# yunjinli/visual-slam

Hardware: AMD Instinct MI355X
Metric: stereo frames/sec, detect+describe (1500 feats) + stereo match, 752x480 (higher is better)
Workload: dtype u8/f32/f64; 1 GPU; synthetic 752x480 stereo, 1500 feats/frame (BASELINE configs[1]); independent streams per GPU (configs[3]); inputs_resident_in_hbm=True, distinct_stereo_pairs_per_gpu=1024, distinct_scenes_per_gpu=64, stereo_frames_per_pass_per_gpu=1024, hip_streams=2, stereo_frames_per_launch=512, num_features=1500, match=threshold 70, ratio 1.2, cross-check

## Files before the change

visual-slam_amd/csrc/detect.hip:

```cpp
#include <type_traits>

#include "vsl_common.h"

#ifndef K1_ROWS
#define K1_ROWS 60
#endif
#ifndef K1_ROWS_SMALL
#define K1_ROWS_SMALL 29
#endif
#define VSL_QUALITY_LEVEL 0.01
#define K1_WLIST 384
#define K1_COLS 60

__device__ __forceinline__ int reflect101(int i, int n) { return i < 0 ? -i : (i >= n ? 2 * n - 2 - i : i); }

struct RowF {
  float rx, ry;
};

struct RowRaw {
  unsigned l, m, r;
};

typedef __amdgpu_buffer_rsrc_t ImgSrd;
__device__ __forceinline__ RowRaw rowload(ImgSrd img, int w, int yr, unsigned xm, unsigned xe, unsigned xp) {
  const int row = yr * w;
  RowRaw o;
  o.l = __builtin_amdgcn_raw_buffer_load_b8(img, (int)xm, row, 0);
  o.m = __builtin_amdgcn_raw_buffer_load_b8(img, (int)xe, row, 0);
  o.r = __builtin_amdgcn_raw_buffer_load_b8(img, (int)xp, row, 0);
  return o;
}

__device__ __forceinline__ RowF rowfilt(RowRaw p, float s, float s2) {
  const float l = (float)p.l, m = (float)p.m, r = (float)p.r;
  RowF o;
  o.rx = r - l;
  float t = s * l;
  t = t + s2 * m;
  t = t + s * r;
  o.ry = t;
  return o;
}

__device__ __forceinline__ float from_lane_below(float v) {
  return __builtin_bit_cast(float, __builtin_amdgcn_update_dpp(0, __builtin_bit_cast(int, v), 0x138, 0xf, 0xf, true));
}
__device__ __forceinline__ float from_lane_above(float v) {
  return __builtin_bit_cast(float, __builtin_amdgcn_update_dpp(0, __builtin_bit_cast(int, v), 0x130, 0xf, 0xf, true));
}

__device__ __forceinline__ double dpp_below_f64(double v) {
  const uint64_t b = __builtin_bit_cast(uint64_t, v);
  const uint32_t lo = (uint32_t)__builtin_amdgcn_update_dpp(0, (int)(uint32_t)b, 0x138, 0xf, 0xf, true);
  const uint32_t hi = (uint32_t)__builtin_amdgcn_update_dpp(0, (int)(uint32_t)(b >> 32), 0x138, 0xf, 0xf, true);
  return __builtin_bit_cast(double, ((uint64_t)hi << 32) | lo);
}

__device__ __forceinline__ double dpp_above_f64(double v) {
  const uint64_t b = __builtin_bit_cast(uint64_t, v);
  const uint32_t lo = (uint32_t)__builtin_amdgcn_update_dpp(0, (int)(uint32_t)b, 0x130, 0xf, 0xf, true);
  const uint32_t hi = (uint32_t)__builtin_amdgcn_update_dpp(0, (int)(uint32_t)(b >> 32), 0x130, 0xf, 0xf, true);
  return __builtin_bit_cast(double, ((uint64_t)hi << 32) | lo);
}

__device__ __forceinline__ float fmax3(float a, float b, float c) {
  float r;
  asm("v_max3_f32 %0, %1, %2, %3" : "=v"(r) : "v"(a), "v"(b), "v"(c));
  return r;
}

__device__ __forceinline__ float fmax2(float a, float b) {
  float r;
  asm("v_max_f32 %0, %1, %2" : "=v"(r) : "v"(a), "v"(b));
  return r;
}

#define K1_SQRT_FLOOR 0x1p-100f
__device__ __forceinline__ float fast_sqrt_rn(float t) {
  const float y = __builtin_amdgcn_rsqf(__builtin_fmaxf(t, K1_SQRT_FLOOR));
  const float r = t * y;
  const float e = __builtin_fmaf(-r, r, t);
  return __builtin_fmaf(e, 0.5f * y, r);
}
__device__ __forceinline__ float sqrt_rn(float t) {
  float r = fast_sqrt_rn(t);
  const bool small = t < K1_SQRT_FLOOR;
  if (__builtin_amdgcn_ballot_w64(small) != 0ull) {
    asm volatile("" ::: "memory");
    const bool rare = small && t > 0.f;
    if (__builtin_amdgcn_ballot_w64(rare) != 0ull) {
      asm volatile("" ::: "memory");
      if (rare) r = sqrtf(t);
    }
  }
  return r;
}

__global__ void sqrt_check_kernel(uint32_t lo, uint32_t hi, unsigned long long* bad) {
  const uint64_t stride = (uint64_t)gridDim.x * blockDim.x;
  unsigned long long n = 0;
  for (uint64_t b = (uint64_t)lo + blockIdx.x * blockDim.x + threadIdx.x; b <= hi; b += stride) {
    const float t = __builtin_bit_cast(float, (uint32_t)b);
    n += __builtin_bit_cast(uint32_t, fast_sqrt_rn(t)) != __builtin_bit_cast(uint32_t, sqrtf(t));
  }
  if (n) atomicAdd(bad, n);
}

__global__ void detect_init_kernel(int32_t* meta, int first, int n) {
  const int i = blockIdx.x * blockDim.x + threadIdx.x;
  if (i < n) {
    meta[(size_t)(first + i) * VSL_META_STRIDE + VSL_META_MAX] = INT32_MIN;
    meta[(size_t)(first + i) * VSL_META_STRIDE + VSL_META_NCAND] = 0;
  }
}

template <bool STORE_RESPONSE, int ROWS>
__global__ __launch_bounds__(256) void min_eig_response_kernel(const uint8_t* __restrict__ images,
                                                               float* __restrict__ response, int32_t* __restrict__ meta,
                                                               uint64_t* __restrict__ cand, size_t cand_cap, int w, int h,
                                                               int first, int wlist_cap, int n_images, int tiles_x, int tiles_y) {
  __shared__ uint64_t list[4][K1_WLIST];
  __shared__ int wave_n[4], wave_max[4], g_base;
  __shared__ double xbuf[4][2][66];
  const int tiles = tiles_x * tiles_y;
  int img_i, tile;
  if (n_images >= 8) {
    const int xcd = blockIdx.x & 7, sl = blockIdx.x >> 3;
    img_i = (sl / tiles) * 8 + xcd;
    tile = sl - (sl / tiles) * tiles;
  } else {
    img_i = blockIdx.x / tiles;
    tile = blockIdx.x - img_i * tiles;
  }
  if (img_i >= n_images) return;
  const int bx = tile % tiles_x, by = tile / tiles_x;
  const int slot = first + img_i;
  const ImgSrd img = __builtin_amdgcn_make_buffer_rsrc((void*)(images + (size_t)slot * w * h), 0, w * h, 0x00020000);
  float* __restrict__ resp = response + (size_t)slot * w * h;
  const int lane = threadIdx.x & 63;
  const int wave = __builtin_amdgcn_readfirstlane(threadIdx.x >> 6);
  const int xs = bx * K1_COLS;
  const int y0 = (by * 4 + wave) * ROWS;
  int n_wave = 0;
  int own_max = INT32_MIN;
  if (y0 < h) {
    const float s = (float)(1.0 / (4.0 * 3.0 * 255.0));
    const float s2 = 2.0f * s;
    const int x = xs - 2 + lane;
    const unsigned xe = (unsigned)reflect101(min(max(x, -1), w), w);
    const unsigned xm = (unsigned)reflect101((int)xe - 1, w), xp = (unsigned)reflect101((int)xe + 1, w);
    const bool own_col = lane >= 2 && lane < 2 + K1_COLS && x < w;
    const bool cand_col = own_col && x >= 1 && x < w - 1;
    const unsigned long long cand_lanes = __builtin_amdgcn_ballot_w64(cand_col);

    struct R3 {
      double xx, xy, yy;
    };
    R3 ra = {0, 0, 0}, rb = ra, bs = ra;
    float va = 0.f, vb = 0.f, hA = 0.f, hB = 0.f, hC = 0.f;
    RowF fA = {0.f, 0.f}, fB = fA, fC = fA;
    int prev_ye = -100, pre_row = -100;
    RowRaw pre = {0u, 0u, 0u};
    float vmax = -3.0e38f;
    const int y_end = min(h, y0 + ROWS);
    auto step = [&](auto steady_tag, auto even_tag, int q, R3& r2, R3& r1, float& v_mid_slot, float& v_dn_slot, float& h_up,
                    float& h_mid, float& h_dn, RowF& f0, RowF& f1, RowF& f2) {
      constexpr bool STEADY = decltype(steady_tag)::value;
      constexpr bool EVEN = decltype(even_tag)::value;
      if (STEADY) {
        f2 = rowfilt(pre, s, s2);
        pre = rowload(img, w, min(q + 2, h - 1), xm, xe, xp);
      } else {
        const int ye = reflect101(min(max(q, -1), h), h);
        if (ye == prev_ye + 1 && ye + 1 < h) {
          if (pre_row != ye + 1) pre = rowload(img, w, ye + 1, xm, xe, xp);
          f2 = rowfilt(pre, s, s2);
        } else {
          f0 = rowfilt(rowload(img, w, reflect101(ye - 1, h), xm, xe, xp), s, s2);
          f1 = rowfilt(rowload(img, w, ye, xm, xe, xp), s, s2);
          f2 = rowfilt(rowload(img, w, reflect101(ye + 1, h), xm, xe, xp), s, s2);
        }
        pre_row = min(ye + 2, h - 1);
        pre = rowload(img, w, pre_row, xm, xe, xp);
        prev_ye = ye;
      }
      const float dx = (f0.rx + f2.rx) * s + f1.rx * s2;
      const float dy = f2.ry - f0.ry;
      const double dxx = (double)(dx * dx), dxy = (double)(dx * dy), dyy = (double)(dy * dy);
      R3 cur;
      {
        xbuf[wave][0][lane + 1] = dxx;
        xbuf[wave][1][lane + 1] = dxy;
        asm volatile("" ::: "memory");
        const double lxx = xbuf[wave][0][lane], uxx = xbuf[wave][0][lane + 2];
        const double lxy = xbuf[wave][1][lane], uxy = xbuf[wave][1][lane + 2];
        asm volatile("" ::: "memory");
        cur.xx = (lxx + dxx) + uxx;
        cur.xy = (lxy + dxy) + uxy;
        cur.yy = (dpp_below_f64(dyy) + dyy) + dpp_above_f64(dyy);
      }
      const int y = q - 1;
      double Axx, Axy, Ayy;
      if (EVEN) {
        bs.xx = r1.xx + cur.xx;
        bs.xy = r1.xy + cur.xy;
        bs.yy = r1.yy + cur.yy;
        Axx = r2.xx + bs.xx;
        Axy = r2.xy + bs.xy;
        Ayy = r2.yy + bs.yy;
      } else {
        Axx = bs.xx + cur.xx;
        Axy = bs.xy + cur.xy;
        Ayy = bs.yy + cur.yy;
      }
      r2 = cur;
      const float X = (float)Axx, b = (float)Axy, Y = (float)Ayy;
      const float xpy = X + Y, d = 0.5f * (X - Y);
      float t = d * d;
      t = t + b * b;
      const float v_dn = __builtin_fmaf(0.5f, xpy, -sqrt_rn(t));
      float h_tmp;
      asm volatile("s_nop 1\n\tv_max_f32_dpp %0, %2, %2 wave_shr:1 row_mask:0xf bank_mask:0xf bound_ctrl:0\n\t"
                   "v_max_f32_dpp %1, %2, %0 wave_shl:1 row_mask:0xf bank_mask:0xf bound_ctrl:0"
                   : "=&v"(h_tmp), "=&v"(h_dn)
                   : "v"(v_dn));
      if (own_col && y >= y0 && y < y_end) {
        if (STORE_RESPONSE) resp[y * w + x] = v_dn;
        vmax = fmax2(vmax, v_dn);
      }
      const float v_mid = v_mid_slot;
      const int yc = q - 2;
      if (yc >= y0 && yc < y_end && yc >= 1 && yc < h - 1) {
        const float m9 = fmax3(h_up, h_mid, h_dn);
        const bool ge0 = v_mid >= m9;
        if ((__builtin_amdgcn_ballot_w64(ge0) & cand_lanes) != 0ull) {
          const bool ge = ge0 && v_mid > 0.f;
          const unsigned long long mask = __builtin_amdgcn_ballot_w64(ge) & cand_lanes;
          if (cand_col && ge) {
            const uint32_t ob = (uint32_t)vsl_float_to_ordered(v_mid) ^ 0x80000000u;
            const uint64_t key = ((uint64_t)ob << 32) | ((uint32_t)yc << 16) | (uint32_t)x;
            const int p = n_wave + (int)__builtin_amdgcn_mbcnt_hi((uint32_t)(mask >> 32),
                                                                  __builtin_amdgcn_mbcnt_lo((uint32_t)mask, 0u));
            if (__builtin_expect(p < wlist_cap, 1)) {
              list[wave][p] = key;
            } else {
              const int g = atomicAdd(&meta[(size_t)slot * VSL_META_STRIDE + VSL_META_NCAND], 1);
              if ((size_t)g < cand_cap) cand[(size_t)slot * cand_cap + g] = key;
            }
          }
          n_wave += __popcll(mask);
        }
      }
      v_dn_slot = v_dn;
    };
    const int q_first = y0 - 2, q_last = y_end + 1;
    typedef std::integral_constant<bool, true> Steady;
    typedef std::integral_constant<bool, false> Generic;
    typedef std::integral_constant<bool, true> Even;
    typedef std::integral_constant<bool, false> Odd;
#define K1_STEP_E0(T, q) step(T{}, Even{}, q, ra, rb, va, vb, hA, hB, hC, fA, fB, fC)
#define K1_STEP_O1(T, q) step(T{}, Odd{}, q, rb, ra, vb, va, hB, hC, hA, fB, fC, fA)
#define K1_STEP_E2(T, q) step(T{}, Even{}, q, ra, rb, va, vb, hC, hA, hB, fC, fA, fB)
#define K1_STEP_O3(T, q) step(T{}, Odd{}, q, rb, ra, vb, va, hA, hB, hC, fA, fB, fC)
#define K1_STEP_E4(T, q) step(T{}, Even{}, q, ra, rb, va, vb, hB, hC, hA, fB, fC, fA)
#define K1_STEP_O5(T, q) step(T{}, Odd{}, q, rb, ra, vb, va, hC, hA, hB, fC, fA, fB)
    constexpr int K1_OPEN = (ROWS + 4) % 6;
    static_assert(K1_OPEN == 3 || K1_OPEN == 4, "opening sequence written for 3 or 4 steps");
#define K1_STRIP(T)                                \
  K1_STEP_E0(Generic, q_first);                    \
  K1_STEP_O1(T, q_first + 1);                      \
  K1_STEP_E2(T, q_first + 2);                      \
  if constexpr (K1_OPEN == 3) {                    \
    for (int q = q_first + 3; q <= q_last; q += 6) { \
      K1_STEP_O3(T, q);                            \
      K1_STEP_E4(T, q + 1);                        \
      K1_STEP_O5(T, q + 2);                        \
      K1_STEP_E0(T, q + 3);                        \
      K1_STEP_O1(T, q + 4);                        \
      K1_STEP_E2(T, q + 5);                        \
    }                                              \
  } else {                                         \
    K1_STEP_O3(T, q_first + 3);                    \
    for (int q = q_first + 4; q <= q_last; q += 6) { \
      K1_STEP_E4(T, q);                            \
      K1_STEP_O5(T, q + 1);                        \
      K1_STEP_E0(T, q + 2);                        \
      K1_STEP_O1(T, q + 3);                        \
      K1_STEP_E2(T, q + 4);                        \
      K1_STEP_O3(T, q + 5);                        \
    }                                              \
  }
    if (q_first >= 1 && q_last + 1 < h) {
      K1_STRIP(Steady)
    } else {
      K1_STRIP(Generic)
    }
#undef K1_STRIP
#undef K1_STEP_E0
#undef K1_STEP_O1
#undef K1_STEP_E2
#undef K1_STEP_O3
#undef K1_STEP_E4
#undef K1_STEP_O5
#pragma unroll
    for (int o = 32; o > 0; o >>= 1) vmax = fmaxf(vmax, __shfl_xor(vmax, o));
    own_max = vsl_float_to_ordered(vmax);
    if (lane == 0) atomicMax(&meta[(size_t)slot * VSL_META_STRIDE + VSL_META_MAX], own_max);
  }
  if (lane == 0) wave_max[wave] = own_max;
  __syncthreads();
  int kept = min(n_wave, wlist_cap);
  {
    const float wg_max = vsl_ordered_to_float(max(max(wave_max[0], wave_max[1]), max(wave_max[2], wave_max[3])));
    if (wg_max > 0.f && kept > 0) {
      const float thr = (float)((double)wg_max * VSL_QUALITY_LEVEL);
      const uint32_t floor_hi = (uint32_t)vsl_float_to_ordered(thr) ^ 0x80000000u;
      const int have = kept;
      kept = 0;
      for (int i0 = 0; i0 < have; i0 += 64) {
        const int i = i0 + lane;
        const uint64_t key = i < have ? list[wave][i] : 0ull;
        const bool keep = i < have && (uint32_t)(key >> 32) > floor_hi;
        const unsigned long long m = __builtin_amdgcn_ballot_w64(keep);
        if (keep) list[wave][kept + (int)__builtin_amdgcn_mbcnt_hi((uint32_t)(m >> 32), __builtin_amdgcn_mbcnt_lo((uint32_t)m, 0u))] = key;
        kept += __popcll(m);
      }
    }
  }
  if (lane == 0) wave_n[wave] = kept;
  __syncthreads();
  const int c0 = wave_n[0], c1 = wave_n[1], c2 = wave_n[2], c3 = wave_n[3];
  const int n = c0 + c1 + c2 + c3;
  if (n == 0) return;
  if (threadIdx.x == 0) g_base = atomicAdd(&meta[(size_t)slot * VSL_META_STRIDE + VSL_META_NCAND], n);
  __syncthreads();
  const int base = g_base + (wave > 0 ? c0 : 0) + (wave > 1 ? c1 : 0) + (wave > 2 ? c2 : 0);
  const int mine = wave_n[wave];
  for (int i = lane; i < mine; i += 64)
    if ((size_t)(base + i) < cand_cap) cand[(size_t)slot * cand_cap + base + i] = list[wave][i];
}

#define SEL_THREADS 1024
#define SEL_CHUNK 8192
#define SEL_EMPTY 0xFFFFFFFFu
#define SEL_BINS 1024
#define SEL_MAX_BLOCKERS 6
static_assert(SEL_THREADS <= 1024 && SEL_MAX_BLOCKERS * 10 <= 64, "blocker packing");

struct SelShared {
  int wave_tot[16];
  int hist[256];
  unsigned long long sel_prefix;
  int sel_k;
  int n_chunk;
};

__device__ __forceinline__ int block_scan(bool p, int* wave_tot, int& total) {
  const int lane = threadIdx.x & 63, wave = threadIdx.x >> 6;
  const unsigned long long m = __ballot(p);
  const int within = __popcll(m & ((1ull << lane) - 1ull));
  __syncthreads();
  if (lane == 0) wave_tot[wave] = __popcll(m);
  __syncthreads();
  int off = 0, tot = 0;
#pragma unroll
  for (int w = 0; w < 16; w++) {
    const int v = wave_tot[w];
    off += (w < wave) ? v : 0;
    tot += v;
  }
  total = tot;
  return off + within;
}

#define SEL_MAX_CELLS 6144
#define SEL_KEYS_PADDED (SEL_CHUNK + SEL_CHUNK / 32)
#define SEL_PHYS(i) ((i) + ((i) >> 5))
#define SEL_LDS_BYTES (SEL_KEYS_PADDED * 8 + SEL_MAX_CELLS * 2 * 4 + SEL_THREADS * 4 * 3 + SEL_MAX_CELLS * 4 + 2048)
static_assert(SEL_LDS_BYTES <= 160 * 1024, "selection kernel LDS budget");

template <int LOGK>
__device__ __forceinline__ void sel_sort_blocked(uint64_t* keys, int tid, int log_n) {
  constexpr int KPT = 1 << LOGK;
  for (int m = 1; m <= log_n; m++) {
    const int k = 1 << m;
    for (int top = m - 1; top >= 0;) {
      const int b = top >= LOGK - 1 ? top - (LOGK - 1) : 0;
      const int nb = top - b + 1;
      const int t_hi = tid >> b, t_lo = tid & ((1 << b) - 1);
      const int i0 = (t_hi << (b + LOGK)) | t_lo;
      uint64_t rk[KPT];
#pragma unroll
      for (int r = 0; r < KPT; r++) rk[r] = keys[SEL_PHYS(i0 | (r << b))];
#pragma unroll
      for (int x = LOGK - 1; x >= 0; x--) {
        if (x < nb) {
#pragma unroll
          for (int r = 0; r < KPT; r++) {
            if ((r & (1 << x)) == 0) {
              const bool desc = ((i0 | (r << b)) & k) == 0;
              const uint64_t u = rk[r], v = rk[r | (1 << x)];
              const bool sw = desc ? (u < v) : (u > v);
              rk[r] = sw ? v : u;
              rk[r | (1 << x)] = sw ? u : v;
            }
          }
        }
      }
#pragma unroll
      for (int r = 0; r < KPT; r++) keys[SEL_PHYS(i0 | (r << b))] = rk[r];
      __syncthreads();
      top = b - 1;
    }
  }
}

template <bool GRID_GLOBAL>
__global__ __launch_bounds__(SEL_THREADS) void select_kernel(const uint64_t* __restrict__ cand_all,
                                                             int32_t* meta,
                                                             int32_t* __restrict__ kp_xy, int32_t* __restrict__ kp_count,
                                                             int w, int h, size_t cand_cap, int F, int first,
                                                             int num_features, int border, double quality,
                                                             uint32_t* __restrict__ grid_scratch, int bucket_cap) {
  __shared__ __align__(16) unsigned char smem[GRID_GLOBAL ? (SEL_KEYS_PADDED * 8 + SEL_THREADS * 4 * 3 + 2048) : SEL_LDS_BYTES];
  const int slot = first + blockIdx.x;
  const uint64_t* __restrict__ cand = cand_all + (size_t)slot * cand_cap;
  const int n_cand_raw = meta[(size_t)slot * VSL_META_STRIDE + VSL_META_NCAND];
  const int n_cand = min(n_cand_raw, (int)cand_cap);
  const int gw = (w + 7) / 8 + 2, gh = (h + 7) / 8 + 2, cells = (gw * gh + 1) & ~1;
  uint64_t* keys = (uint64_t*)smem;
  SelShared* sh = (SelShared*)(keys + SEL_KEYS_PADDED);
  volatile uint32_t* acc = GRID_GLOBAL ? (volatile uint32_t*)(grid_scratch + (size_t)slot * cells * 3) : (volatile uint32_t*)(sh + 1);
  volatile int* head = (volatile int*)(acc + 2 * (size_t)cells);
  int* next = GRID_GLOBAL ? (int*)(sh + 1) : (int*)(head + cells);
  unsigned long long* node = (unsigned long long*)next;
  int* state = next + 2 * SEL_THREADS;
  const int tid = threadIdx.x;

  for (int i = tid; i < 2 * cells; i += SEL_THREADS) acc[i] = SEL_EMPTY;
  for (int i = tid; i < cells; i += SEL_THREADS) head[i] = -1;
  __syncthreads();

  int n_acc = 0, n_out = 0;
  unsigned long long hi = ~0ull;
  int32_t* out = kp_xy + (size_t)slot * F * 2;
  const float maxv = vsl_ordered_to_float(meta[(size_t)slot * VSL_META_STRIDE + VSL_META_MAX]);
  const float thr = (float)((double)maxv * quality);
  const unsigned long long floor_key =
      (((unsigned long long)((uint32_t)vsl_float_to_ordered(thr) ^ 0x80000000u)) << 32) | 0xFFFFFFFFull;
  int remaining = 0;
  int* bcount = next;
  int* bstart = next + SEL_THREADS;
  int* bcursor = next + 2 * SEL_THREADS;
  static_assert(SEL_BINS == SEL_THREADS, "one bin per thread");
  const uint32_t hi_max = (uint32_t)vsl_float_to_ordered(maxv) ^ 0x80000000u;
  const uint32_t hi_floor = (uint32_t)vsl_float_to_ordered(thr) ^ 0x80000000u;
  int bshift = 16;
  while (bshift < 31 && (hi_max >> bshift) - (hi_floor >> bshift) >= (uint32_t)SEL_BINS) bshift++;
  const uint32_t bin_top = hi_max >> bshift;
  bool bucket_sort = false;
  if (maxv > 0.f) {
    bcount[tid] = 0;
    if (tid == 0) sh->n_chunk = 0;
    __syncthreads();
    for (int i = tid; i < n_cand; i += SEL_THREADS) {
      const unsigned long long key = cand[i];
      if (key > floor_key) {
        const uint32_t kb = min((uint32_t)(key >> 32) >> bshift, bin_top);
        atomicAdd(&bcount[bin_top - kb], 1);
      }
    }
    __syncthreads();
    const int c = bcount[tid];
    int x = c;
    const int lane = tid & 63, wv = tid >> 6;
#pragma unroll
    for (int o = 1; o < 64; o <<= 1) {
      const int y = __shfl_up(x, o);
      if (lane >= o) x += y;
    }
    int cmax = c;
#pragma unroll
    for (int o = 32; o > 0; o >>= 1) cmax = max(cmax, __shfl_xor(cmax, o));
    if (lane == 63) sh->wave_tot[wv] = x;
    if (lane == 0) sh->hist[wv] = cmax;
    __syncthreads();
    int off = 0, fullest = 0;
    remaining = 0;
#pragma unroll
    for (int k = 0; k < 16; k++) {
      off += k < wv ? sh->wave_tot[k] : 0;
      remaining += sh->wave_tot[k];
      fullest = max(fullest, sh->hist[k]);
    }
    bstart[tid] = off + x - c;
    bcursor[tid] = 0;
    bucket_sort = remaining <= SEL_CHUNK && fullest <= bucket_cap;
    __syncthreads();
  }

  while (remaining > 0 && n_acc < num_features) {
    unsigned long long lo = 0;
    if (remaining > SEL_CHUNK) {
      unsigned long long prefix = 0;
      int k = SEL_CHUNK;
      for (int shift = 56; shift >= 0; shift -= 8) {
        for (int i = tid; i < 256; i += SEL_THREADS) sh->hist[i] = 0;
        __syncthreads();
        const unsigned long long pmask = shift == 56 ? 0ull : (~0ull << (shift + 8));
        for (int i = tid; i < n_cand; i += SEL_THREADS) {
          const unsigned long long key = cand[i];
          if (key < hi && key > floor_key && (key & pmask) == prefix) atomicAdd(&sh->hist[(int)((key >> shift) & 255)], 1);
        }
        __syncthreads();
        if (tid == 0) {
          int kk = k, d = 255;
          for (; d > 0; d--) {
            if (sh->hist[d] >= kk) break;
            kk -= sh->hist[d];
          }
          sh->sel_k = kk;
          sh->sel_prefix = prefix | ((unsigned long long)d << shift);
        }
        __syncthreads();
        k = sh->sel_k;
        prefix = sh->sel_prefix;
        __syncthreads();
      }
      lo = prefix;
    }
    int n_chunk;
    if (bucket_sort) {
      for (int i = tid; i < n_cand; i += SEL_THREADS) {
        const unsigned long long key = cand[i];
        if (key > floor_key) {
          const int bin = (int)(bin_top - min((uint32_t)(key >> 32) >> bshift, bin_top));
          const int p = bstart[bin] + atomicAdd(&bcursor[bin], 1);
          keys[SEL_PHYS(p)] = key;
        }
      }
      __syncthreads();
      n_chunk = remaining;
      unsigned long long mykey[SEL_CHUNK / SEL_THREADS];
      int mypos[SEL_CHUNK / SEL_THREADS];
#pragma unroll
      for (int k = 0; k < SEL_CHUNK / SEL_THREADS; k++) {
        const int p = tid + SEL_THREADS * k;
        mypos[k] = -1;
        if (p < n_chunk) {
          const unsigned long long key = keys[SEL_PHYS(p)];
          const int bin = (int)(bin_top - min((uint32_t)(key >> 32) >> bshift, bin_top));
          const int s0 = bstart[bin], e0 = s0 + bcount[bin];
          int larger = 0;
          for (int q = s0; q < e0; q++) larger += keys[SEL_PHYS(q)] > key;
          mykey[k] = key;
          mypos[k] = s0 + larger;
        }
      }
      __syncthreads();
#pragma unroll
      for (int k = 0; k < SEL_CHUNK / SEL_THREADS; k++)
        if (mypos[k] >= 0) keys[SEL_PHYS(mypos[k])] = mykey[k];
      __syncthreads();
      bucket_sort = false;
    } else {
      if (tid == 0) sh->n_chunk = 0;
      __syncthreads();
      for (int i = tid; i < n_cand; i += SEL_THREADS) {
        const unsigned long long key = cand[i];
        if (key >= lo && key < hi && key > floor_key) {
          const int p = atomicAdd(&sh->n_chunk, 1);
          if (p < SEL_CHUNK) keys[SEL_PHYS(p)] = key;
        }
      }
      __syncthreads();
      n_chunk = min(sh->n_chunk, SEL_CHUNK);
      int N = 1024;
      while (N < n_chunk) N <<= 1;
      for (int i = n_chunk + tid; i < N; i += SEL_THREADS) keys[SEL_PHYS(i)] = 0ull;
      __syncthreads();
      if (N >= 2048) {
        if (N == 8192) sel_sort_blocked<3>(keys, tid, 13);
        else if (N == 4096) sel_sort_blocked<2>(keys, tid, 12);
        else sel_sort_blocked<1>(keys, tid, 11);
      } else {
        for (int k = 2; k <= N; k <<= 1) {
          for (int j = k >> 1; j > 0; j >>= 1) {
            for (int t = tid; t < (N >> 1); t += SEL_THREADS) {
              const int i = ((t & ~(j - 1)) << 1) | (t & (j - 1));
              const int l = i | j;
              const uint64_t a = keys[SEL_PHYS(i)], b = keys[SEL_PHYS(l)];
              const bool desc = (i & k) == 0;
              if (desc ? (a < b) : (a > b)) {
                keys[SEL_PHYS(i)] = b;
                keys[SEL_PHYS(l)] = a;
              }
            }
            __syncthreads();
          }
        }
      }
    }
    for (int r0 = 0; r0 < n_chunk && n_acc < num_features; r0 += SEL_THREADS) {
      const int r = r0 + tid;
      int px = 0, py = 0, cell = 0, cx = 0, cy = 0;
      bool alive = false;
      if (r < n_chunk) {
        const uint32_t pix = (uint32_t)(keys[SEL_PHYS(r)] & 0xFFFFFFFFull);
        py = (int)(pix >> 16);
        px = (int)(pix & 0xFFFFu);
        cx = (px >> 3) + 1;
        cy = (py >> 3) + 1;
        cell = cy * gw + cx;
        alive = true;
        uint32_t a18[18];
#pragma unroll
        for (int k = 0; k < 9; k++) {
          const int c2 = cell + (k / 3 - 1) * gw + (k % 3 - 1);
          const unsigned long long two = *(volatile const unsigned long long*)&acc[2 * c2];
          a18[2 * k] = (uint32_t)two;
          a18[2 * k + 1] = (uint32_t)(two >> 32);
        }
        int near = 0;
#pragma unroll
        for (int k = 0; k < 18; k++) {
          const uint32_t a = a18[k];
          const int dx = px - (int)(a & 0xFFFF), dy = py - (int)(a >> 16);
          const unsigned d2 = (unsigned)(dx * dx) + (unsigned)(dy * dy);
          near |= (int)(a != SEL_EMPTY) & (int)(d2 < 64u);
        }
        alive = near == 0;
      }
      state[tid] = alive ? 0 : 2;
      {
        const int nxt = alive ? atomicExch((int*)&head[cell], tid) : -1;
        node[tid] = ((unsigned long long)(uint32_t)nxt << 32) | ((uint32_t)px | ((uint32_t)py << 16));
      }
      __syncthreads();
      int nb = 0;
      unsigned long long blk = 0ull;
      if (alive) {
        int h9[9];
#pragma unroll
        for (int k = 0; k < 9; k++) h9[k] = head[cell + (k / 3 - 1) * gw + (k % 3 - 1)];
#pragma unroll
        for (int k = 0; k < 9; k++)
          for (int u = h9[k]; u >= 0;) {
            const unsigned long long nd = node[u];
            const int uu = u;
            u = (int)(nd >> 32);
            if (uu < tid) {
              const uint32_t q = (uint32_t)nd;
              const int dx = px - (int)(q & 0xFFFF), dy = py - (int)(q >> 16);
              if (dx * dx + dy * dy < 64) {
                blk = (blk << 10) | (unsigned long long)(unsigned)uu;
                nb++;
              }
            }
          }
      }
      bool undecided = alive;
      while (__ballot(undecided) != 0ull) {
        if (undecided) {
          bool rej = false, blocked = false;
          if (nb <= SEL_MAX_BLOCKERS) {
#pragma unroll
            for (int k = 0; k < SEL_MAX_BLOCKERS; k++)
              if (k < nb) {
                const int su = ((volatile int*)state)[(int)(blk >> (10 * k)) & 1023];
                rej = rej || (su == 1);
                blocked = blocked || (su == 0);
              }
          } else {
            for (int k = 0; k < 9; k++)
                for (int u = head[cell + (k / 3 - 1) * gw + (k % 3 - 1)], un = -1; u >= 0; u = un) {
                  const unsigned long long nd = node[u];
                  un = (int)(nd >> 32);
                  if (u < tid) {
                    const uint32_t q = (uint32_t)nd;
                    const int dx = px - (int)(q & 0xFFFF), dy = py - (int)(q >> 16);
                    if (dx * dx + dy * dy < 64) {
                      const int su = ((volatile int*)state)[u];
                      rej = rej || (su == 1);
                      blocked = blocked || (su == 0);
                    }
                  }
                }
          }
          const int ns = rej ? 2 : (blocked ? 0 : 1);
          if (ns) {
            ((volatile int*)state)[tid] = ns;
            undecided = false;
          }
        }
        __builtin_amdgcn_s_sleep(1);
      }
      __syncthreads();
      const bool accepted = alive && state[tid] == 1;
      int total = 0;
      const int rank = n_acc + block_scan(accepted, sh->wave_tot, total);
      const bool keep = accepted && rank < num_features;
      const bool inb = keep && px >= border && px < w - border && py >= border && py < h - border;
      int total_out = 0;
      const int pos = n_out + block_scan(inb, sh->wave_tot, total_out);
      if (inb) {
        out[2 * pos] = px;
        out[2 * pos + 1] = py;
      }
      if (keep) {
        const uint32_t packed = (uint32_t)px | ((uint32_t)py << 16);
        if (atomicCAS((uint32_t*)&acc[2 * cell], SEL_EMPTY, packed) != SEL_EMPTY) atomicCAS((uint32_t*)&acc[2 * cell + 1], SEL_EMPTY, packed);
      }
      if (alive) head[cell] = -1;
      n_acc = min(num_features, n_acc + total);
      n_out += total_out;
      __syncthreads();
    }
    hi = lo;
    remaining -= n_chunk;
  }
  if (tid == 0) {
    kp_count[slot] = n_out;
    meta[(size_t)slot * VSL_META_STRIDE + VSL_META_NCAND_LAST] = n_cand_raw;
    meta[(size_t)slot * VSL_META_STRIDE + VSL_META_MAX] = INT32_MIN;
    meta[(size_t)slot * VSL_META_STRIDE + VSL_META_NCAND] = 0;
  }
}

extern "C" int vsl_diag_sqrt_check(vsl_ctx* ctx, uint32_t lo_bits, uint32_t hi_bits, unsigned long long* n_mismatch) {
  if (!ctx || !n_mismatch || lo_bits > hi_bits || hi_bits > 0x7f7fffffu)
    return vsl_fail(ctx, VSL_ERR_INVALID, "vsl_diag_sqrt_check: bad range");
  VSL_HIP(ctx, hipSetDevice(ctx->device));
  void* d = nullptr;
  int rc = vsl_ctx_dscratch(ctx, sizeof(unsigned long long), &d);
  if (rc) return rc;
  VSL_HIP(ctx, hipMemsetAsync(d, 0, sizeof(unsigned long long), ctx->stream));
  hipLaunchKernelGGL(sqrt_check_kernel, dim3(4096), dim3(256), 0, ctx->stream, lo_bits, hi_bits, (unsigned long long*)d);
  VSL_CHECK_LAUNCH(ctx);
  VSL_HIP(ctx, hipMemcpyAsync(n_mismatch, d, sizeof(unsigned long long), hipMemcpyDeviceToHost, ctx->stream));
  VSL_HIP(ctx, hipStreamSynchronize(ctx->stream));
  return VSL_OK;
}

int vsl_launch_detect(vsl_ctx* ctx, vsl_frames* f, int first, int n, int num_features) {
  if (n <= 0) return VSL_OK;
  if (num_features < 1 || num_features > f->F)
    return vsl_fail(ctx, VSL_ERR_INVALID, "num_features %d not in [1, %d]", num_features, f->F);
  static_assert(sizeof(SelShared) <= 2048, "SelShared fits its LDS slot");
  const int cells = (((f->w + 7) / 8 + 2) * ((f->h + 7) / 8 + 2) + 1) & ~1;
  const bool grid_global = cells > SEL_MAX_CELLS;
  if (grid_global && !f->sel_grid) {
    VSL_HIP(ctx, hipMalloc((void**)&f->sel_grid, sizeof(uint32_t) * 3 * (size_t)cells * f->max_images));
  }
  const int w = f->w, h = f->h;
  {
    VslStage st(ctx, VSL_STAGE_RESPONSE);
    if (f->detect_meta_dirty)
      hipLaunchKernelGGL(detect_init_kernel, dim3((f->max_images + 255) / 256), dim3(256), 0, ctx->stream, f->meta, 0, f->max_images);
    f->detect_meta_dirty = true;
    const bool small = n < 8 && !f->store_response;
    const int rows = small ? K1_ROWS_SMALL : K1_ROWS;
    const int tiles_y = (h + 4 * rows - 1) / (4 * rows);
    const int tiles_x = (w + K1_COLS - 1) / K1_COLS;
    const dim3 k1_grid((unsigned)(tiles_x * tiles_y) * (unsigned)(n >= 8 ? 8 * ((n + 7) / 8) : n));
    const int wcap = ctx->k1_list_cap < 0 ? K1_WLIST : min(ctx->k1_list_cap, K1_WLIST);
    if (f->store_response)
      hipLaunchKernelGGL((min_eig_response_kernel<true, K1_ROWS>), k1_grid, dim3(256), 0, ctx->stream, f->images, f->response, f->meta,
                         f->cand, f->cand_cap, w, h, first, wcap, n, tiles_x, tiles_y);
    else if (small)
      hipLaunchKernelGGL((min_eig_response_kernel<false, K1_ROWS_SMALL>), k1_grid, dim3(256), 0, ctx->stream, f->images, f->response, f->meta,
                         f->cand, f->cand_cap, w, h, first, wcap, n, tiles_x, tiles_y);
    else
      hipLaunchKernelGGL((min_eig_response_kernel<false, K1_ROWS>), k1_grid, dim3(256), 0, ctx->stream, f->images, f->response, f->meta,
                         f->cand, f->cand_cap, w, h, first, wcap, n, tiles_x, tiles_y);
    VSL_CHECK_LAUNCH(ctx);
  }
  {
    VslStage st(ctx, VSL_STAGE_SELECT);
    if (grid_global)
      hipLaunchKernelGGL(select_kernel<true>, dim3(n), dim3(SEL_THREADS), 0, ctx->stream, f->cand, f->meta, f->kp_xy,
                         f->kp_count, w, h, f->cand_cap, f->F, first, num_features, 19, VSL_QUALITY_LEVEL, f->sel_grid, ctx->select_bucket_cap);
    else
      hipLaunchKernelGGL(select_kernel<false>, dim3(n), dim3(SEL_THREADS), 0, ctx->stream, f->cand, f->meta, f->kp_xy,
                         f->kp_count, w, h, f->cand_cap, f->F, first, num_features, 19, VSL_QUALITY_LEVEL, (uint32_t*)nullptr,
                         ctx->select_bucket_cap);
    VSL_CHECK_LAUNCH(ctx);
  }
  f->detect_meta_dirty = false;
  return VSL_OK;
}
```

Before: 366,300 frames/s.

## Shrink selection-kernel LDS footprint to co-reside with describe workgroups

```diff
diff --git a/visual-slam_amd/csrc/detect.hip b/visual-slam_amd/csrc/detect.hip
--- a/visual-slam_amd/csrc/detect.hip
+++ b/visual-slam_amd/csrc/detect.hip
@@ -343,7 +343,6 @@
 
 #define SEL_THREADS 1024
 #define SEL_CHUNK 8192
-#define SEL_EMPTY 0xFFFFFFFFu
 #define SEL_BINS 1024
 #define SEL_MAX_BLOCKERS 6
 static_assert(SEL_THREADS <= 1024 && SEL_MAX_BLOCKERS * 10 <= 64, "blocker packing");
@@ -357,37 +356,70 @@
 };
 
 __device__ __forceinline__ int block_scan(bool p, int* wave_tot, int& total) {
-  const int lane = threadIdx.x & 63, wave = threadIdx.x >> 6;
+  const int lane = threadIdx.x & 63, wave = __builtin_amdgcn_readfirstlane(threadIdx.x >> 6);
   const unsigned long long m = __ballot(p);
-  const int within = __popcll(m & ((1ull << lane) - 1ull));
+  const int within = (int)__builtin_amdgcn_mbcnt_hi((uint32_t)(m >> 32), __builtin_amdgcn_mbcnt_lo((uint32_t)m, 0u));
+  const int mine = __popcll(m);
   __syncthreads();
-  if (lane == 0) wave_tot[wave] = __popcll(m);
+  if (lane == 0) wave_tot[wave] = mine;
   __syncthreads();
-  int off = 0, tot = 0;
-#pragma unroll
-  for (int w = 0; w < 16; w++) {
-    const int v = wave_tot[w];
-    off += (w < wave) ? v : 0;
-    tot += v;
-  }
-  total = tot;
-  return off + within;
+  int x = wave_tot[lane & 15];
+  x += __builtin_amdgcn_update_dpp(0, x, 0x111, 0xf, 0xf, true);
+  x += __builtin_amdgcn_update_dpp(0, x, 0x112, 0xf, 0xf, true);
+  x += __builtin_amdgcn_update_dpp(0, x, 0x114, 0xf, 0xf, true);
+  x += __builtin_amdgcn_update_dpp(0, x, 0x118, 0xf, 0xf, true);
+  total = __builtin_amdgcn_readlane(x, 15);
+  return __builtin_amdgcn_readlane(x, wave) - mine + within;
 }
 
 #define SEL_MAX_CELLS 6144
+#define SEL_ACC_VALID 0x40u
+#define SEL_HEAD_EMPTY 0xFFFFu
 #define SEL_KEYS_PADDED (SEL_CHUNK + SEL_CHUNK / 32)
 #define SEL_PHYS(i) ((i) + ((i) >> 5))
-#define SEL_LDS_BYTES (SEL_KEYS_PADDED * 8 + SEL_MAX_CELLS * 2 * 4 + SEL_THREADS * 4 * 3 + SEL_MAX_CELLS * 4 + 2048)
-static_assert(SEL_LDS_BYTES <= 160 * 1024, "selection kernel LDS budget");
-
-template <int LOGK>
-__device__ __forceinline__ void sel_sort_blocked(uint64_t* keys, int tid, int log_n) {
+#define SEL_GRID_BYTES (SEL_MAX_CELLS * 2 * 2)
+#define SEL_STAGE_PAD (SEL_CHUNK * 4 - SEL_THREADS * 4 - SEL_GRID_BYTES)
+#define SEL_LDS_BYTES (SEL_KEYS_PADDED * 8 + 2048 + SEL_THREADS * 4 * 3 + SEL_GRID_BYTES + SEL_STAGE_PAD)
+static_assert(SEL_STAGE_PAD >= 0, "ranking staging array");
+static_assert(SEL_LDS_BYTES <= 160 * 1024 - 39344, "selection kernel LDS budget: one describe_tile_kernel workgroup fits beside it");
+
+__device__ __forceinline__ uint32_t sel_xchg16(volatile uint16_t* arr, int idx, uint32_t v) {
+  uint32_t* word = (uint32_t*)arr + (idx >> 1);
+  const int s = (idx & 1) * 16;
+  uint32_t old = *(volatile uint32_t*)word;
+  for (;;) {
+    const uint32_t got = atomicCAS(word, old, (old & ~(0xFFFFu << s)) | (v << s));
+    if (got == old) break;
+    old = got;
+  }
+  return (old >> s) & 0xFFFFu;
+}
+
+__device__ __forceinline__ int sel_head_rank(uint32_t h) { return h == SEL_HEAD_EMPTY ? -1 : (int)h; }
+
+__device__ __forceinline__ void sel_acc_insert(volatile uint16_t* arr, int idx, uint32_t b) {
+  uint32_t* word = (uint32_t*)arr + (idx >> 1);
+  const int s = (idx & 1) * 16;
+  uint32_t old = *(volatile uint32_t*)word;
+  for (;;) {
+    const uint32_t cur = (old >> s) & 0xFFFFu;
+    if ((cur & 0xFF00u) != 0u) break;
+    const uint32_t got = atomicCAS(word, old, old | (b << (s + ((cur & 0xFFu) ? 8 : 0))));
+    if (got == old) break;
+    old = got;
+  }
+}
+
+template <int LOGK, int REPS>
+__device__ __forceinline__ void sel_sort_blocked(uint64_t* keys, int tid0, int log_n) {
   constexpr int KPT = 1 << LOGK;
   for (int m = 1; m <= log_n; m++) {
     const int k = 1 << m;
     for (int top = m - 1; top >= 0;) {
       const int b = top >= LOGK - 1 ? top - (LOGK - 1) : 0;
       const int nb = top - b + 1;
+#pragma unroll 1
+      for (int tid = tid0; tid < REPS * SEL_THREADS; tid += SEL_THREADS) {
       const int t_hi = tid >> b, t_lo = tid & ((1 << b) - 1);
       const int i0 = (t_hi << (b + LOGK)) | t_lo;
       uint64_t rk[KPT];
@@ -410,6 +442,7 @@
       }
 #pragma unroll
       for (int r = 0; r < KPT; r++) keys[SEL_PHYS(i0 | (r << b))] = rk[r];
+      }
       __syncthreads();
       top = b - 1;
     }
@@ -423,24 +456,21 @@
                                                              int w, int h, size_t cand_cap, int F, int first,
                                                              int num_features, int border, double quality,
                                                              uint32_t* __restrict__ grid_scratch, int bucket_cap) {
-  __shared__ __align__(16) unsigned char smem[GRID_GLOBAL ? (SEL_KEYS_PADDED * 8 + SEL_THREADS * 4 * 3 + 2048) : SEL_LDS_BYTES];
+  __shared__ __align__(16) unsigned char smem[SEL_LDS_BYTES];
   const int slot = first + blockIdx.x;
   const uint64_t* __restrict__ cand = cand_all + (size_t)slot * cand_cap;
   const int n_cand_raw = meta[(size_t)slot * VSL_META_STRIDE + VSL_META_NCAND];
   const int n_cand = min(n_cand_raw, (int)cand_cap);
   const int gw = (w + 7) / 8 + 2, gh = (h + 7) / 8 + 2, cells = (gw * gh + 1) & ~1;
   uint64_t* keys = (uint64_t*)smem;
-  SelShared* sh = (SelShared*)(keys + SEL_KEYS_PADDED);
-  volatile uint32_t* acc = GRID_GLOBAL ? (volatile uint32_t*)(grid_scratch + (size_t)slot * cells * 3) : (volatile uint32_t*)(sh + 1);
-  volatile int* head = (volatile int*)(acc + 2 * (size_t)cells);
-  int* next = GRID_GLOBAL ? (int*)(sh + 1) : (int*)(head + cells);
+  uint32_t* keys32 = (uint32_t*)smem;
+  SelShared* sh = (SelShared*)(smem + SEL_KEYS_PADDED * 8);
+  int* next = (int*)(smem + SEL_KEYS_PADDED * 8 + 2048);
+  volatile uint16_t* acc = GRID_GLOBAL ? (volatile uint16_t*)(grid_scratch + (size_t)slot * cells) : (volatile uint16_t*)(next + 3 * SEL_THREADS);
+  volatile uint16_t* head = acc + cells;
   unsigned long long* node = (unsigned long long*)next;
   int* state = next + 2 * SEL_THREADS;
   const int tid = threadIdx.x;
-
-  for (int i = tid; i < 2 * cells; i += SEL_THREADS) acc[i] = SEL_EMPTY;
-  for (int i = tid; i < cells; i += SEL_THREADS) head[i] = -1;
-  __syncthreads();
 
   int n_acc = 0, n_out = 0;
   unsigned long long hi = ~0ull;
@@ -453,6 +483,7 @@
   int* bcount = next;
   int* bstart = next + SEL_THREADS;
   int* bcursor = next + 2 * SEL_THREADS;
+  uint32_t* stage = (uint32_t*)bcursor;
   static_assert(SEL_BINS == SEL_THREADS, "one bin per thread");
   const uint32_t hi_max = (uint32_t)vsl_float_to_ordered(maxv) ^ 0x80000000u;
   const uint32_t hi_floor = (uint32_t)vsl_float_to_ordered(thr) ^ 0x80000000u;
@@ -499,6 +530,11 @@
     bucket_sort = remaining <= SEL_CHUNK && fullest <= bucket_cap;
     __syncthreads();
   }
+  if (!bucket_sort) {
+    for (int i = tid; i < cells; i += SEL_THREADS) ((volatile uint32_t*)acc)[i] = i < (cells >> 1) ? 0u : ~0u;
+    __syncthreads();
+  }
+  bool compact = false;
 
   while (remaining > 0 && n_acc < num_features) {
     unsigned long long lo = 0;
@@ -542,27 +578,20 @@
       }
       __syncthreads();
       n_chunk = remaining;
-      unsigned long long mykey[SEL_CHUNK / SEL_THREADS];
-      int mypos[SEL_CHUNK / SEL_THREADS];
-#pragma unroll
-      for (int k = 0; k < SEL_CHUNK / SEL_THREADS; k++) {
-        const int p = tid + SEL_THREADS * k;
-        mypos[k] = -1;
-        if (p < n_chunk) {
-          const unsigned long long key = keys[SEL_PHYS(p)];
-          const int bin = (int)(bin_top - min((uint32_t)(key >> 32) >> bshift, bin_top));
-          const int s0 = bstart[bin], e0 = s0 + bcount[bin];
-          int larger = 0;
-          for (int q = s0; q < e0; q++) larger += keys[SEL_PHYS(q)] > key;
-          mykey[k] = key;
-          mypos[k] = s0 + larger;
-        }
-      }
-      __syncthreads();
-#pragma unroll
-      for (int k = 0; k < SEL_CHUNK / SEL_THREADS; k++)
-        if (mypos[k] >= 0) keys[SEL_PHYS(mypos[k])] = mykey[k];
-      __syncthreads();
+      for (int p = tid; p < n_chunk; p += SEL_THREADS) {
+        const unsigned long long key = keys[SEL_PHYS(p)];
+        const int bin = (int)(bin_top - min((uint32_t)(key >> 32) >> bshift, bin_top));
+        const int s0 = bstart[bin], e0 = s0 + bcount[bin];
+        int larger = 0;
+        for (int q = s0; q < e0; q++) larger += keys[SEL_PHYS(q)] > key;
+        stage[s0 + larger] = (uint32_t)key;
+      }
+      __syncthreads();
+      for (int p = tid; p < n_chunk; p += SEL_THREADS) keys32[p] = stage[p];
+      __syncthreads();
+      for (int i = tid; i < cells; i += SEL_THREADS) ((volatile uint32_t*)acc)[i] = i < (cells >> 1) ? 0u : ~0u;
+      __syncthreads();
+      compact = true;
       bucket_sort = false;
     } else {
       if (tid == 0) sh->n_chunk = 0;
@@ -581,9 +610,9 @@
       for (int i = n_chunk + tid; i < N; i += SEL_THREADS) keys[SEL_PHYS(i)] = 0ull;
       __syncthreads();
       if (N >= 2048) {
-        if (N == 8192) sel_sort_blocked<3>(keys, tid, 13);
-        else if (N == 4096) sel_sort_blocked<2>(keys, tid, 12);
-        else sel_sort_blocked<1>(keys, tid, 11);
+        if (N == 8192) sel_sort_blocked<2, 2>(keys, tid, 13);
+        else if (N == 4096) sel_sort_blocked<2, 1>(keys, tid, 12);
+        else sel_sort_blocked<1, 1>(keys, tid, 11);
       } else {
         for (int k = 2; k <= N; k <<= 1) {
           for (int j = k >> 1; j > 0; j >>= 1) {
@@ -604,61 +633,61 @@
     }
     for (int r0 = 0; r0 < n_chunk && n_acc < num_features; r0 += SEL_THREADS) {
       const int r = r0 + tid;
-      int px = 0, py = 0, cell = 0, cx = 0, cy = 0;
+      int px = 0, py = 0, cell = 0;
       bool alive = false;
       if (r < n_chunk) {
-        const uint32_t pix = (uint32_t)(keys[SEL_PHYS(r)] & 0xFFFFFFFFull);
+        const uint32_t pix = compact ? keys32[r] : (uint32_t)(keys[SEL_PHYS(r)] & 0xFFFFFFFFull);
         py = (int)(pix >> 16);
         px = (int)(pix & 0xFFFFu);
-        cx = (px >> 3) + 1;
-        cy = (py >> 3) + 1;
-        cell = cy * gw + cx;
-        alive = true;
-        uint32_t a18[18];
-#pragma unroll
-        for (int k = 0; k < 9; k++) {
-          const int c2 = cell + (k / 3 - 1) * gw + (k % 3 - 1);
-          const unsigned long long two = *(volatile const unsigned long long*)&acc[2 * c2];
-          a18[2 * k] = (uint32_t)two;
-          a18[2 * k + 1] = (uint32_t)(two >> 32);
-        }
+        cell = ((py >> 3) + 1) * gw + (px >> 3) + 1;
+        const int lx = px & 7, ly = py & 7;
         int near = 0;
 #pragma unroll
-        for (int k = 0; k < 18; k++) {
-          const uint32_t a = a18[k];
-          const int dx = px - (int)(a & 0xFFFF), dy = py - (int)(a >> 16);
-          const unsigned d2 = (unsigned)(dx * dx) + (unsigned)(dy * dy);
-          near |= (int)(a != SEL_EMPTY) & (int)(d2 < 64u);
+        for (int oy = -1; oy <= 1; oy++) {
+          const int row = cell + oy * gw;
+          const uint32_t t0 = acc[row - 1], t1 = acc[row], t2 = acc[row + 1];
+#pragma unroll
+          for (int k = 0; k < 6; k++) {
+            const uint32_t b = ((k >> 1) == 0 ? t0 : (k >> 1) == 1 ? t1 : t2) >> (8 * (k & 1));
+            const int dx = lx - 8 * ((k >> 1) - 1) - (int)(b & 7u), dy = ly - 8 * oy - (int)((b >> 3) & 7u);
+            const unsigned d2 = (unsigned)(dx * dx) + (unsigned)(dy * dy);
+            near |= (int)((b & SEL_ACC_VALID) != 0u) & (int)(d2 < 64u);
+          }
         }
         alive = near == 0;
       }
       state[tid] = alive ? 0 : 2;
       {
-        const int nxt = alive ? atomicExch((int*)&head[cell], tid) : -1;
+        const uint32_t prev = alive ? sel_xchg16(head, cell, (uint32_t)tid) : SEL_HEAD_EMPTY;
+        const int nxt = sel_head_rank(prev);
         node[tid] = ((unsigned long long)(uint32_t)nxt << 32) | ((uint32_t)px | ((uint32_t)py << 16));
       }
       __syncthreads();
       int nb = 0;
       unsigned long long blk = 0ull;
       if (alive) {
-        int h9[9];
-#pragma unroll
-        for (int k = 0; k < 9; k++) h9[k] = head[cell + (k / 3 - 1) * gw + (k % 3 - 1)];
-#pragma unroll
-        for (int k = 0; k < 9; k++)
-          for (int u = h9[k]; u >= 0;) {
-            const unsigned long long nd = node[u];
-            const int uu = u;
-            u = (int)(nd >> 32);
-            if (uu < tid) {
-              const uint32_t q = (uint32_t)nd;
-              const int dx = px - (int)(q & 0xFFFF), dy = py - (int)(q >> 16);
-              if (dx * dx + dy * dy < 64) {
-                blk = (blk << 10) | (unsigned long long)(unsigned)uu;
-                nb++;
+#pragma unroll 1
+        for (int oy = -1; oy <= 1; oy++) {
+          const int row = cell + oy * gw;
+          uint32_t h3[3];
+#pragma unroll
+          for (int k = 0; k < 3; k++) h3[k] = head[row + k - 1];
+#pragma unroll
+          for (int k = 0; k < 3; k++)
+            for (int u = sel_head_rank(h3[k]); u >= 0;) {
+              const unsigned long long nd = node[u];
+              const int uu = u;
+              u = (int)(nd >> 32);
+              if (uu < tid) {
+                const uint32_t q = (uint32_t)nd;
+                const int dx = px - (int)(q & 0xFFFF), dy = py - (int)(q >> 16);
+                if (dx * dx + dy * dy < 64) {
+                  blk = (blk << 10) | (unsigned long long)(unsigned)uu;
+                  nb++;
+                }
               }
             }
-          }
+        }
       }
       bool undecided = alive;
       while (__ballot(undecided) != 0ull) {
@@ -674,7 +703,7 @@
               }
           } else {
             for (int k = 0; k < 9; k++)
-                for (int u = head[cell + (k / 3 - 1) * gw + (k % 3 - 1)], un = -1; u >= 0; u = un) {
+                for (int u = sel_head_rank(head[cell + (k / 3 - 1) * gw + (k % 3 - 1)]), un = -1; u >= 0; u = un) {
                   const unsigned long long nd = node[u];
                   un = (int)(nd >> 32);
                   if (u < tid) {
@@ -708,11 +737,8 @@
         out[2 * pos] = px;
         out[2 * pos + 1] = py;
       }
-      if (keep) {
-        const uint32_t packed = (uint32_t)px | ((uint32_t)py << 16);
-        if (atomicCAS((uint32_t*)&acc[2 * cell], SEL_EMPTY, packed) != SEL_EMPTY) atomicCAS((uint32_t*)&acc[2 * cell + 1], SEL_EMPTY, packed);
-      }
-      if (alive) head[cell] = -1;
+      if (keep) sel_acc_insert(acc, cell, SEL_ACC_VALID | (uint32_t)((py & 7) << 3) | (uint32_t)(px & 7));
+      if (alive) head[cell] = (uint16_t)SEL_HEAD_EMPTY;
       n_acc = min(num_features, n_acc + total);
       n_out += total_out;
       __syncthreads();
@@ -751,7 +777,7 @@
   const int cells = (((f->w + 7) / 8 + 2) * ((f->h + 7) / 8 + 2) + 1) & ~1;
   const bool grid_global = cells > SEL_MAX_CELLS;
   if (grid_global && !f->sel_grid) {
-    VSL_HIP(ctx, hipMalloc((void**)&f->sel_grid, sizeof(uint32_t) * 3 * (size_t)cells * f->max_images));
+    VSL_HIP(ctx, hipMalloc((void**)&f->sel_grid, sizeof(uint32_t) * (size_t)cells * f->max_images));
   }
   const int w = f->w, h = f->h;
   {
```

After: 370,800 frames/s (median of 6 runs). 1.01x the previous value.
